# samuel-watson/glmmrMCML

Measured on AMD Instinct MI355X. Metric: MCML iters/sec x m chains (simlik evals/sec), higher is better.
Workload: dtype f64

## Files before the change

### glmmrmcml_amd/csrc/band_plan.h

```cpp
#pragma once
#include "common.h"
#include <algorithm>
#include <map>
#include <memory>

namespace mcml {

constexpr int BD_BM = 80, BD_BN = 128, BD_BK = 32, BD_STAGES = 3;
constexpr int BD_A_BYTES = BD_BK * BD_BM * 8;
constexpr int BD_B_BYTES = BD_BK * BD_BN * 8;
constexpr int BD_STAGE_BYTES = BD_A_BYTES + BD_B_BYTES;
constexpr size_t BD_LDS_BYTES = (size_t)BD_STAGES * BD_STAGE_BYTES;
constexpr int BD_NA = 3, BD_NB = 4, BD_PER_TILE = BD_NA + BD_NB;
constexpr int BD_TILE_ELEMS = BD_BM * BD_BN;

struct BandItem { int band, kt0, kt1, slot; };
struct BandRed { int band, s0, s1, pad; };

struct BandPlanDev {
    int gn = 0, nwg = 0, nred = 0, nslots = 0;
    int paired = 0;
    DevBuf items, wg_ptr, red, part;
};

struct SkinnyPlan {
    int nrb = 0, nkc = 0, ldp = 0;
    DevBuf range;
    DevBuf part;
};

struct BandPlan {
    int M = 0, K = 0, nbands = 0;
    std::vector<int> kr;
    long tiles = 0;
    std::map<int, std::unique_ptr<BandPlanDev>> by_gn;
    std::unique_ptr<SkinnyPlan> skinny;

    void reset(int M_, int K_, const std::vector<int>& kr_)
    {
        M = M_; K = K_; kr = kr_; nbands = (M + BD_BM - 1) / BD_BM;
        tiles = 0;
        for (int b = 0; b < nbands; ++b) tiles += kr[2 * b + 1] - kr[2 * b];
        by_gn.clear();
        skinny.reset();
    }

    static bool decompose(const std::vector<int>& kr, int nbands, int gn, int target_wg, std::vector<BandItem>& items,
                          std::vector<int>& wg_ptr, std::vector<BandRed>& red, int& nslots)
    {
        items.clear(); wg_ptr.clear(); red.clear(); nslots = 0;
        const int npairs = (nbands + 1) / 2;
        if ((long)npairs * gn * 5 >= (long)target_wg * 4) {
            for (int p = 0; p < npairs; ++p) {
                wg_ptr.push_back((int)items.size());
                items.push_back({p, kr[2 * p], kr[2 * p + 1], -1});
                const int q = nbands - 1 - p;
                if (q > p) items.push_back({q, kr[2 * q], kr[2 * q + 1], -1});
            }
            wg_ptr.push_back((int)items.size());
            return true;
        }
        int nwg = target_wg / gn; if (nwg < 1) nwg = 1;
        constexpr long OVH = 3;
        auto fill = [&](long cap, bool emit) -> int {
            int used = 1; long room = cap;
            if (emit) wg_ptr.push_back(0);
            for (int b = 0; b < nbands; ++b) {
                int k0 = kr[2 * b]; const int k1 = kr[2 * b + 1];
                const int first = (int)items.size();
                int pieces = 0;
                do {
                    if (room < OVH + 2) { ++used; room = cap; if (emit) wg_ptr.push_back((int)items.size()); }
                    long take = (room - OVH) / 2; if (take > k1 - k0) take = k1 - k0;
                    if (emit) items.push_back({b, k0, k0 + (int)take, -1});
                    k0 += (int)take; room -= OVH + 2 * take; ++pieces;
                } while (k0 < k1);
                if (emit && pieces > 1) {
                    for (int t = 0; t < pieces; ++t) items[first + t].slot = nslots + t;
                    red.push_back({b, nslots, nslots + pieces, 0});
                    nslots += pieces;
                }
            }
            if (emit) wg_ptr.push_back((int)items.size());
            return used;
        };
        long T = 0;
        for (int b = 0; b < nbands; ++b) T += kr[2 * b + 1] - kr[2 * b];
        long lo = OVH + 2, hi = 2 * T + OVH * nbands + OVH + 2;
        while (lo < hi) {
            const long mid = (lo + hi) / 2;
            if (fill(mid, false) <= nwg) hi = mid; else lo = mid + 1;
        }
        fill(lo, true);
        return false;
    }

    int device_plan(int gn, hipStream_t s, BandPlanDev** out)
    {
        auto it = by_gn.find(gn);
        if (it != by_gn.end()) { *out = it->second.get(); return MCML_OK; }
        std::unique_ptr<BandPlanDev> d(new BandPlanDev());
        std::vector<BandItem> items; std::vector<int> wg_ptr; std::vector<BandRed> red; int nslots = 0;
        d->paired = decompose(kr, nbands, gn, 256, items, wg_ptr, red, nslots) ? 1 : 0;
        d->gn = gn; d->nwg = (int)wg_ptr.size() - 1; d->nred = (int)red.size(); d->nslots = nslots;
        MCML_TRY(d->items.ensure(sizeof(BandItem) * (items.size() + 1)));
        MCML_TRY(d->wg_ptr.ensure(sizeof(int) * wg_ptr.size()));
        MCML_HIP(hipMemcpyAsync(d->items.p, items.data(), sizeof(BandItem) * items.size(), hipMemcpyHostToDevice, s));
        MCML_HIP(hipMemcpyAsync(d->wg_ptr.p, wg_ptr.data(), sizeof(int) * wg_ptr.size(), hipMemcpyHostToDevice, s));
        if (nslots > 0) {
            MCML_TRY(d->red.ensure(sizeof(BandRed) * red.size()));
            MCML_HIP(hipMemcpyAsync(d->red.p, red.data(), sizeof(BandRed) * red.size(), hipMemcpyHostToDevice, s));
            MCML_TRY(d->part.ensure(sizeof(double) * (size_t)nslots * gn * BD_TILE_ELEMS));
        }
        MCML_HIP(hipStreamSynchronize(s));
        *out = d.get();
        by_gn[gn] = std::move(d);
        return MCML_OK;
    }
};

}
```

### glmmrmcml_amd/csrc/debug_hooks.hip

```cpp
#include "dgemm_mfma.h"
#include "dgemm_dl.h"
#include "dgemm_band.h"

using namespace mcml;

extern "C" int glmmr_mcml_dbg_dgemm(int M, int N, int K, const double* A, int lda,
                                    const double* B, int ldb, int b_nmajor,
                                    double alpha, double beta, double* C, int ldc,
                                    int lower_only, int force_tile)
{
    int ndev = 0;
    if (hipGetDeviceCount(&ndev) != hipSuccess || ndev == 0) {
        set_error("no HIP device: libglmmr_mcml_hip has no CPU fallback");
        return MCML_ENODEVICE;
    }
    hipStream_t s = nullptr;
    DevMat dA, dB, dC;
    if (force_tile == 40) {
        MCML_REQUIRE(!b_nmajor && !lower_only, "dbg_dgemm: the direct-to-LDS kernel takes a K-major B and all tiles");
        const int kpad = round_up(K, 32);
        MCML_TRY(dA.alloc(M, K, 32));
        MCML_HIP(hipMemset(dA.d(), 0, sizeof(double) * (size_t)dA.ld * dA.cols_alloc));
        MCML_HIP(hipMemcpy2D(dA.d(), sizeof(double) * dA.ld, A, sizeof(double) * lda, sizeof(double) * M, K, hipMemcpyHostToDevice));
        MCML_TRY(dB.alloc(kpad, N));
// ... 45 lines not shown
    auto rnd = [&]() { x ^= x << 13; x ^= x >> 7; x ^= x << 17; return (double)(x >> 11) / 9007199254740992.0 * 2 - 1; };
    for (auto& v : hA) v = rnd();
    for (auto& v : hB) v = rnd();
    DevMat dA, dB, dC;
    MCML_TRY(upload_matrix(dA, hA.data(), M, K, M, s));
    if (b_nmajor) MCML_TRY(upload_matrix(dB, hB.data(), N, K, N, s));
    else MCML_TRY(upload_matrix(dB, hB.data(), K, N, K, s));
    MCML_TRY(upload_matrix(dC, hC.data(), M, N, M, s));
    EpiAxpby epi{dC.d(), dC.ld, beta != 0.0 ? 1e-3 : 1.0, beta};
    const bool lo = lower_only != 0;
    auto go = [&]() {
        if (force_tile >= 20)
            return b_nmajor ? launch_gemm_dl<true>(s, M, N, K, dA.d(), dA.ld, dB.d(), dB.ld, epi, lo, force_tile - 19)
                            : launch_gemm_dl<false>(s, M, N, K, dA.d(), dA.ld, dB.d(), dB.ld, epi, lo, force_tile - 19);
        return b_nmajor ? launch_gemm<true>(s, M, N, K, dA.d(), dA.ld, dB.d(), dB.ld, epi, lo, force_tile)
                        : launch_gemm<false>(s, M, N, K, dA.d(), dA.ld, dB.d(), dB.ld, epi, lo, force_tile);
    };
    for (int i = 0; i < 3; i++) MCML_TRY(go());
    hipEvent_t e0, e1;
    MCML_HIP(hipEventCreate(&e0));
    MCML_HIP(hipEventCreate(&e1));
    MCML_HIP(hipEventRecord(e0, s));
    for (int i = 0; i < iters; i++) MCML_TRY(go());
    MCML_HIP(hipEventRecord(e1, s));
    MCML_HIP(hipEventSynchronize(e1));
    float ms = 0;
    MCML_HIP(hipEventElapsedTime(&ms, e0, e1));
    *ms_per_launch = ms / iters;
    (void)hipEventDestroy(e0);
    (void)hipEventDestroy(e1);
    return MCML_OK;
}

extern "C" int glmmr_mcml_dbg_dgemm_band(int M, int N, int K, const double* A, int lda, const double* B, int ldb,
                                         double* C, int ldc, int* tiles_executed)
{
    int ndev = 0;
    if (hipGetDeviceCount(&ndev) != hipSuccess || ndev == 0) {
        set_error("no HIP device: libglmmr_mcml_hip has no CPU fallback");
        return MCML_ENODEVICE;
    }
    MCML_REQUIRE(M > 0 && N > 0 && K > 0 && A && B && C, "dbg_dgemm_band: bad argument");
    hipStream_t s = nullptr;
    DevMat dA, dB, dC;
    MCML_TRY(dA.alloc(M, K, 32));
    MCML_HIP(hipMemset(dA.d(), 0, sizeof(double) * (size_t)dA.ld * dA.cols_alloc));
    MCML_HIP(hipMemcpy2D(dA.d(), sizeof(double) * dA.ld, A, sizeof(double) * lda, sizeof(double) * M, K, hipMemcpyHostToDevice));
    MCML_TRY(dB.alloc(round_up(K, 32), N));
    MCML_HIP(hipMemset(dB.d(), 0, sizeof(double) * (size_t)dB.ld * N));
    MCML_HIP(hipMemcpy2D(dB.d(), sizeof(double) * dB.ld, B, sizeof(double) * ldb, sizeof(double) * K, N, hipMemcpyHostToDevice));
    MCML_TRY(dC.alloc(M, N));
    MCML_HIP(hipMemset(dC.d(), 0, sizeof(double) * (size_t)dC.ld * N));
    MCML_REQUIRE(dlds_applicable(M, N, K, dA.d(), dA.ld, dA.cols_alloc, dB.d(), dB.ld), "dbg_dgemm_band: contract");
    const int nbands = (M + BD_BM - 1) / BD_BM;
    DevBuf kr;
    MCML_TRY(kr.ensure(sizeof(int) * 2 * nbands));
    hipLaunchKernelGGL(k_band_ranges, dim3(nbands), dim3(256), 0, s, dA.d(), dA.ld, M, K, kr.as<int>());
    MCML_HIP(hipGetLastError());
    std::vector<int> hk(2 * nbands);
    MCML_HIP(hipMemcpy(hk.data(), kr.p, sizeof(int) * 2 * nbands, hipMemcpyDeviceToHost));
    BandPlan plan;
    plan.reset(M, K, hk);
    if (tiles_executed) *tiles_executed = (int)plan.tiles;
    EpiAxpby epi{dC.d(), dC.ld, 1.0, 0.0};
    MCML_TRY(launch_gemm_band(s, plan, N, dA.d(), dA.ld, dB.d(), dB.ld, epi));
    MCML_TRY(download_matrix(C, ldc, dC.d(), dC.ld, M, N, s));
    return MCML_OK;
}

extern "C" int glmmr_mcml_dbg_band_clocks(int M, int N, int iters, int mode, double* out3)
{
    int ndev = 0;
    if (hipGetDeviceCount(&ndev) != hipSuccess || ndev == 0) {
        set_error("no HIP device: libglmmr_mcml_hip has no CPU fallback");
        return MCML_ENODEVICE;
    }
    hipStream_t s = nullptr;
    if (getenv("GLMMR_MCML_DBG_STREAM")) MCML_HIP(hipStreamCreateWithFlags(&s, hipStreamNonBlocking));
    std::vector<double> hA((size_t)M * M, 0.0), hB((size_t)M * N);
    uint64_t x = 88172645463325252ULL;
    auto rnd = [&]() { x ^= x << 13; x ^= x >> 7; x ^= x << 17; return (double)(x >> 11) / 9007199254740992.0 * 2 - 1; };
    const bool cst = getenv("GLMMR_MCML_DBG_DATA") && !strcmp(getenv("GLMMR_MCML_DBG_DATA"), "const");
    const bool dec = getenv("GLMMR_MCML_DBG_DATA") && !strcmp(getenv("GLMMR_MCML_DBG_DATA"), "decay");
    for (int j = 0; j < M; ++j) for (int i = j; i < M; ++i) hA[i + (size_t)j * M] = cst ? 1.0 : dec ? rnd() * std::exp(-(double)(i - j) / 40.0) : rnd();
    for (auto& v : hB) v = cst ? 1.0 : rnd();
    DevMat dA, dB, dC;
    MCML_TRY(dA.alloc(M, M, 32));
    MCML_HIP(hipMemset(dA.d(), 0, sizeof(double) * (size_t)dA.ld * dA.cols_alloc));
    MCML_HIP(hipMemcpy2D(dA.d(), sizeof(double) * dA.ld, hA.data(), sizeof(double) * M, sizeof(double) * M, M, hipMemcpyHostToDevice));
    MCML_TRY(dB.alloc(round_up(M, 32), N));
    MCML_HIP(hipMemset(dB.d(), 0, sizeof(double) * (size_t)dB.ld * N));
    MCML_HIP(hipMemcpy2D(dB.d(), sizeof(double) * dB.ld, hB.data(), sizeof(double) * M, sizeof(double) * M, N, hipMemcpyHostToDevice));
    MCML_TRY(dC.alloc(M, N));
    const int nbands = (M + BD_BM - 1) / BD_BM;
    DevBuf kr, clk;
    MCML_TRY(kr.ensure(sizeof(int) * 2 * nbands));
    MCML_TRY(clk.ensure(16));
    MCML_HIP(hipMemset(clk.p, 0, 16));
    hipLaunchKernelGGL(k_band_ranges, dim3(nbands), dim3(256), 0, s, dA.d(), dA.ld, M, M, kr.as<int>());
    std::vector<int> hk(2 * nbands);
    MCML_HIP(hipMemcpy(hk.data(), kr.p, sizeof(int) * 2 * nbands, hipMemcpyDeviceToHost));
    BandPlan plan;
    plan.reset(M, M, hk);
    const double tiles = (double)plan.tiles;
    EpiAxpby epi{dC.d(), dC.ld, 1.0, 0.0};
    if (mode < 0) {
        for (int i = 0; i < 3; i++)
            MCML_TRY((launch_gemm_band<EpiAxpby, false>(s, plan, N, dA.d(), dA.ld, dB.d(), dB.ld, epi)));
        hipEvent_t f0, f1;
        MCML_HIP(hipEventCreate(&f0));
        MCML_HIP(hipEventCreate(&f1));
        MCML_HIP(hipEventRecord(f0, s));
        for (int i = 0; i < iters; i++)
            MCML_TRY((launch_gemm_band<EpiAxpby, false>(s, plan, N, dA.d(), dA.ld, dB.d(), dB.ld, epi)));
        MCML_HIP(hipEventRecord(f1, s));
        MCML_HIP(hipEventSynchronize(f1));
        float fms = 0;
        MCML_HIP(hipEventElapsedTime(&fms, f0, f1));
        out3[0] = fms / iters; out3[1] = 0;
        out3[2] = 2.0 * 80.0 * 32.0 * tiles * N / (fms / iters * 1e-3) / 1e12;
        (void)hipEventDestroy(f0);
        (void)hipEventDestroy(f1);
        return MCML_OK;
    }
    if (mode & 16) {
        BandPlanDev* d = nullptr;
        MCML_TRY(plan.device_plan((N + BD_BN - 1) / BD_BN, s, &d));
        const int nb = d->nwg * d->gn;
        DevBuf st;
        MCML_TRY(st.ensure(sizeof(unsigned long long) * (8 + 8 * (size_t)nb)));
        for (int rep = 0; rep < 3; ++rep) {
            MCML_HIP(hipMemset(st.p, 0, sizeof(unsigned long long) * (8 + 8 * (size_t)nb)));
            MCML_TRY((launch_gemm_band<EpiAxpby, true>(s, plan, N, dA.d(), dA.ld, dB.d(), dB.ld, epi, st.as<unsigned long long>(), mode)));
            MCML_HIP(hipDeviceSynchronize());
        }
        std::vector<unsigned long long> h(8 + 8 * (size_t)nb);
// ... 167 lines not shown
```

### glmmrmcml_amd/csrc/dgemm_band.h

```cpp
#pragma once
#include "dgemm_dlds.h"
#include "band_plan.h"

namespace mcml {

struct BandP {
    GemmP g;
    const BandItem* items;
    const int* wg_ptr;
    int nwg;
    double* part;
    int mode;
    unsigned long long* clocks;
};

static __global__ __launch_bounds__(256) void k_band_ranges(const double* A, int lda, int M, int K, int* krange)
{
    __shared__ int smin[256], smax[256];
    const int band = blockIdx.x, r0 = band * BD_BM;
    const int rows = (M - r0 < BD_BM) ? (M - r0) : BD_BM;
    int kmin = 1 << 30, kmax = -1;
    for (int k = threadIdx.x; k < K; k += 256) {
        const double* col = A + r0 + (size_t)k * lda;
        bool nz = false;
        for (int r = 0; r < rows; ++r) nz |= (col[r] != 0.0);
        if (nz) { kmin = min(kmin, k); kmax = max(kmax, k); }
    }
    smin[threadIdx.x] = kmin; smax[threadIdx.x] = kmax;
    __syncthreads();
    for (int o = 128; o > 0; o >>= 1) {
        if ((int)threadIdx.x < o) {
            smin[threadIdx.x] = min(smin[threadIdx.x], smin[threadIdx.x + o]);
            smax[threadIdx.x] = max(smax[threadIdx.x], smax[threadIdx.x + o]);
        }
        __syncthreads();
    }
    if (threadIdx.x == 0) {
        if (smax[0] < 0) { krange[2 * band] = 0; krange[2 * band + 1] = 0; }
        else { krange[2 * band] = smin[0] / BD_BK; krange[2 * band + 1] = smax[0] / BD_BK + 1; }
    }
}

#if defined(__HIP_DEVICE_COMPILE__)
#define BD_RD(dst, addr, off) asm volatile("ds_read_b64 %0, %1 offset:%2" : "=v"(dst) : "v"(addr), "i"(off))
#else
#define BD_RD(dst, addr, off) (dst = 0.0)
#endif
template <int KS>
__device__ __forceinline__ void bd_read(double (&a)[5], double& b, unsigned aaddr, unsigned baddr)
{
    BD_RD(a[0], aaddr, KS * 4 * BD_BM * 8);
    BD_RD(a[1], aaddr, KS * 4 * BD_BM * 8 + 128);
    BD_RD(a[2], aaddr, KS * 4 * BD_BM * 8 + 256);
    BD_RD(a[3], aaddr, KS * 4 * BD_BM * 8 + 384);
    BD_RD(a[4], aaddr, KS * 4 * BD_BM * 8 + 512);
    BD_RD(b, baddr, KS * 2 * BD_BN * 16);
}
template <int LEAVE>
__device__ __forceinline__ void bd_wait(double (&a)[5], double& b)
{
#if defined(__HIP_DEVICE_COMPILE__)
    if constexpr (LEAVE == 6)
        asm volatile("s_waitcnt lgkmcnt(6)" : "+v"(a[0]), "+v"(a[1]), "+v"(a[2]), "+v"(a[3]), "+v"(a[4]), "+v"(b));
    else
        asm volatile("s_waitcnt lgkmcnt(0)" : "+v"(a[0]), "+v"(a[1]), "+v"(a[2]), "+v"(a[3]), "+v"(a[4]), "+v"(b));
#endif
}
__device__ __forceinline__ void bd_mfma(d4 (&acc)[5][1], const double (&a)[5], double b)
{
#pragma unroll
    for (int i = 0; i < 5; ++i) acc[i][0] = __builtin_amdgcn_mfma_f64_16x16x4f64(b, a[i], acc[i][0], 0, 0, 0);
}
// ... 1 lines not shown
template <class Epi, bool DBG>
__global__ __launch_bounds__(512) void dgemm_band_kernel(BandP bp, Epi epi)
{
    const GemmP& p = bp.g;
    extern __shared__ __attribute__((aligned(16))) double smem[];
    char* lds = reinterpret_cast<char*>(smem);
    const int tid = threadIdx.x, lane = tid & 63, wave = __builtin_amdgcn_readfirstlane(tid >> 6);
    const int l15 = lane & 15, lk = lane >> 4;
    unsigned long long t0c = 0, t0r = 0;
    if constexpr (DBG)
        if (bp.clocks && blockIdx.x == 0 && tid == 0) { t0c = __builtin_amdgcn_s_memtime(); t0r = __builtin_amdgcn_s_memrealtime(); }

    const int nblk = bp.nwg * p.gn;
    const int bid = blockIdx.x;
    const int q8 = nblk >> 3, r8 = nblk & 7, xcd = bid & 7;
    const int nid = (xcd < r8 ? xcd * (q8 + 1) : r8 * (q8 + 1) + (xcd - r8) * q8) + (bid >> 3);
    const int pw = nid / p.gn, bj = nid - pw * p.gn;
    const int n0 = bj * BD_BN;

    unsigned vob[BD_NB]; int lb[BD_NB];
#pragma unroll
    for (int s = 0; s < BD_NB; ++s) {
        const int c = wave + 8 * s;
        const int kp = c >> 1, n = ((c & 1) << 6) + lane;
        int gn = n0 + n;
        if (gn >= p.N) gn = 0;
        vob[s] = (unsigned)((2 * kp + (size_t)gn * p.ldb) * 8);
        lb[s] = BD_A_BYTES + c * 1024;
    }
    const size_t stepA = (size_t)BD_BK * p.lda * 8;

    const int it0 = bp.wg_ptr[pw], it1 = bp.wg_ptr[pw + 1];
    BandItem item{0, 0, 0, -1};
    int m0 = 0;
    unsigned voa[BD_NA]; int la[BD_NA];
#pragma unroll
    for (int s = 0; s < BD_NA; ++s) {
        int c = wave + 8 * s;
        if (c >= 20) c = wave + 8;
        la[s] = c * 1024;
    }
    const char* sA = nullptr; const char* sB = nullptr;
    auto load_item = [&](int it) {
#if defined(__HIP_DEVICE_COMPILE__)
        {
            typedef int i4s __attribute__((ext_vector_type(4)));
            i4s raw;
            const BandItem* ip = bp.items + it;
            asm volatile("s_load_dwordx4 %0, %1, 0x0\n\ts_waitcnt lgkmcnt(0)" : "=&s"(raw) : "s"(ip) : "memory");
            item.band = raw.x; item.kt0 = raw.y; item.kt1 = raw.z; item.slot = raw.w;
        }
#else
        item = bp.items[it];
#endif
        m0 = item.band * BD_BM;
#pragma unroll
        for (int s = 0; s < BD_NA; ++s) {
            int c = wave + 8 * s;
            if (c >= 20) c = wave + 8;
            const int o = c * 1024 + lane * 16;
            const int k = o / (BD_BM * 8), m = (o - k * BD_BM * 8) >> 3;
            int gm = m0 + m;
            if (gm >= p.M) gm = 0;
            voa[s] = (unsigned)((gm + (size_t)k * p.lda) * 8);
        }
        sA = reinterpret_cast<const char*>(p.A) + (size_t)item.kt0 * stepA;
        sB = reinterpret_cast<const char*>(p.B) + (size_t)item.kt0 * (BD_BK * 8);
    };
    auto issue = [&](int stage) {
#if defined(__HIP_DEVICE_COMPILE__)
        const unsigned lbase = (unsigned)(size_t)(lds_ptr_t)lds + stage * BD_STAGE_BYTES;
#pragma unroll
        for (int s = 0; s < BD_NA; ++s)
            asm volatile("s_mov_b32 m0, %0\n\ts_nop 0\n\tglobal_load_lds_dwordx4 %1, %2"
                         :: "s"(lbase + la[s]), "v"(voa[s]), "s"(sA) : "memory", "m0");
#pragma unroll
        for (int s = 0; s < BD_NB; ++s)
            asm volatile("s_mov_b32 m0, %0\n\ts_nop 0\n\tglobal_load_lds_dwordx4 %1, %2"
                         :: "s"(lbase + lb[s]), "v"(vob[s]), "s"(sB) : "memory", "m0");
        sA += stepA;
        sB += BD_BK * 8;
#else
        (void)stage; (void)stepA; (void)sA; (void)sB;
#endif
    };
    auto wait_leave = [&](int tiles) {
        static_assert(BD_PER_TILE == 7, "vmcnt immediates below");
        if (tiles >= 2) asm volatile("s_waitcnt vmcnt(14)" ::: "memory");
        else if (tiles == 1) asm volatile("s_waitcnt vmcnt(7)" ::: "memory");
        else asm volatile("s_waitcnt vmcnt(0)" ::: "memory");
    };
    const int mode = DBG ? (bp.mode & 15) : 0;
    const bool stamps = DBG && (bp.mode & 16) && bp.clocks;
    auto stamp = [&](int i) {
        if constexpr (DBG)
            if (stamps && tid == 0) bp.clocks[8 + 8 * (size_t)blockIdx.x + i] = __builtin_amdgcn_s_memrealtime();
    };
    stamp(0);
    bool first_item = true;
    bool pre = false;
    int issued = 0;
    if (it0 < it1) load_item(it0);
    for (int it = it0; it < it1;) {
        const int band = item.band, e_m0 = m0, slot = item.slot;
        const int nk = item.kt1 - item.kt0;

        d4 acc[5][1];
#pragma unroll
        for (int i = 0; i < 5; ++i) acc[i][0] = d4{0.0, 0.0, 0.0, 0.0};

        if (nk > 0 && mode == 0) {
            const unsigned lds0 = (unsigned)(size_t)(lds_ptr_t)lds;
            const unsigned aoff = lds0 + lk * (BD_BM * 8) + l15 * 8;
            const unsigned boff = lds0 + BD_A_BYTES + (((lk >> 1) * BD_BN + wave * 16 + l15) << 4) + ((lk & 1) << 3);
            if (!pre) { issued = 0; for (; issued < BD_STAGES - 1 && issued < nk; ++issued) issue(issued); }
            wait_leave(issued - 1);
            __builtin_amdgcn_s_barrier();
            if (first_item) stamp(1);
            int st = 0;
            double ra[2][5], rb[2];
            bd_read<0>(ra[0], rb[0], aoff, boff);
            for (int kt = 0; kt < nk; ++kt) {
                if (issued < nk) {
                    int sn = st + BD_STAGES - 1; if (sn >= BD_STAGES) sn -= BD_STAGES;
                    issue(sn);
                    ++issued;
                }
                const unsigned aaddr = aoff + st * BD_STAGE_BYTES, baddr = boff + st * BD_STAGE_BYTES;
                int stn = st + 1; if (stn >= BD_STAGES) stn = 0;
#define BD_STEP(KS, CUR, NXT)                                   \
                bd_read<KS + 1>(ra[NXT], rb[NXT], aaddr, baddr); \
                bd_wait<6>(ra[CUR], rb[CUR]);                    \
                bd_mfma(acc, ra[CUR], rb[CUR]);                  \
                __builtin_amdgcn_sched_barrier(0);
                BD_STEP(0, 0, 1) BD_STEP(1, 1, 0) BD_STEP(2, 0, 1) BD_STEP(3, 1, 0)
                BD_STEP(4, 0, 1) BD_STEP(5, 1, 0) BD_STEP(6, 0, 1)
#undef BD_STEP
                wait_leave(issued - kt - 2);
                bd_wait<0>(ra[1], rb[1]);
                __builtin_amdgcn_s_barrier();
                if (kt + 1 < nk) bd_read<0>(ra[0], rb[0], aoff + stn * BD_STAGE_BYTES, boff + stn * BD_STAGE_BYTES);
                bd_mfma(acc, ra[1], rb[1]);
                __builtin_amdgcn_sched_barrier(0);
                st = stn;
            }
        } else if (DBG && nk > 0 && mode == 8) {
            int issued = 0;
            for (; issued < BD_STAGES - 1 && issued < nk; ++issued) issue(issued);
            wait_leave(issued - 1);
            __builtin_amdgcn_s_barrier();
            int st = 0;
            for (int kt = 0; kt < nk; ++kt) {
                if (issued < nk) {
                    int sn = st + BD_STAGES - 1; if (sn >= BD_STAGES) sn -= BD_STAGES;
                    issue(sn);
                    ++issued;
                }
                const double* as = reinterpret_cast<const double*>(lds + st * BD_STAGE_BYTES);
                const double* bs = reinterpret_cast<const double*>(lds + st * BD_STAGE_BYTES + BD_A_BYTES);
#pragma unroll
                for (int ks = 0; ks < BD_BK / 4; ++ks) {
                    const int kk = 4 * ks + lk;
                    double a[5];
#pragma unroll
                    for (int i = 0; i < 5; ++i) a[i] = as[kk * BD_BM + 16 * i + l15];
                    const double b = bs[((kk >> 1) * BD_BN + wave * 16 + l15) * 2 + (kk & 1)];
#pragma unroll
                    for (int i = 0; i < 5; ++i)
                        acc[i][0] = __builtin_amdgcn_mfma_f64_16x16x4f64(b, a[i], acc[i][0], 0, 0, 0);
                }
                wait_leave(issued - kt - 2);
                __builtin_amdgcn_s_barrier();
                st = st + 1; if (st >= BD_STAGES) st = 0;
            }
        } else if (DBG && nk > 0) {
            int issued = 0;
            if (!(mode & 1)) {
                for (; issued < BD_STAGES - 1 && issued < nk; ++issued) issue(issued);
// ... 19 lines not shown
                        b = bs[((kk >> 1) * BD_BN + wave * 16 + l15) * 2 + (kk & 1)];
                    }
#pragma unroll
                    for (int i = 0; i < 5; ++i)
                        acc[i][0] = __builtin_amdgcn_mfma_f64_16x16x4f64(b, a[i], acc[i][0], 0, 0, 0);
                }
                if (!(mode & 1)) wait_leave(issued - kt - 2);
                if (!(mode & 2)) __builtin_amdgcn_s_barrier();
                st = st + 1; if (st >= BD_STAGES) st = 0;
            }
        }
        if (first_item) stamp(2);
        ++it;
        pre = false;
        if (it < it1) {
            load_item(it);
            const int nkn = item.kt1 - item.kt0;
            if (mode == 0 && nk > 0 && nkn > 0) {
                issued = 0;
                for (; issued < BD_STAGES - 1 && issued < nkn; ++issued) issue(issued);
                pre = true;
            }
        }
        if (slot < 0) {
            epi(acc, e_m0, n0 + wave * 16, lane, p.M, p.N, band);
        } else {
            double* P = bp.part + ((size_t)slot * p.gn + bj) * BD_TILE_ELEMS + (size_t)wave * (20 * 64) + lane;
#pragma unroll
            for (int i = 0; i < 5; ++i)
#pragma unroll
                for (int r = 0; r < 4; ++r) P[(i * 4 + r) * 64] = acc[i][0][r];
        }
        if (first_item) { stamp(3); first_item = false; }
        if (!pre) __builtin_amdgcn_s_barrier();
    }
    if constexpr (DBG)
        if (stamps) { asm volatile("s_waitcnt vmcnt(0)" ::: "memory"); stamp(4); }
    if constexpr (DBG)
        if (bp.clocks && blockIdx.x == 0 && tid == 0) {
            atomicAdd(bp.clocks, __builtin_amdgcn_s_memtime() - t0c);
            atomicAdd(bp.clocks + 1, __builtin_amdgcn_s_memrealtime() - t0r);
        }
}

template <class Epi>
__global__ __launch_bounds__(128) void k_band_reduce(const BandRed* red, const double* part, int gn, int M, int N, Epi epi)
{
    const BandRed rd = red[blockIdx.x];
    const int bj = blockIdx.y;
    const int lane = threadIdx.x & 63, wave = blockIdx.z * 2 + (threadIdx.x >> 6);
    d4 acc[5][1];
#pragma unroll
    for (int i = 0; i < 5; ++i) acc[i][0] = d4{0.0, 0.0, 0.0, 0.0};
    const size_t pstride = (size_t)gn * BD_TILE_ELEMS;
    const double* P0 = part + ((size_t)rd.s0 * gn + bj) * BD_TILE_ELEMS + (size_t)wave * (20 * 64) + lane;
    for (int s = rd.s0; s < rd.s1; s += 4) {
        double v[4][20];
#pragma unroll
        for (int u = 0; u < 4; ++u) {
            const double* P = P0 + (size_t)(s - rd.s0 + (s + u < rd.s1 ? u : 0)) * pstride;
#pragma unroll
            for (int t = 0; t < 20; ++t) v[u][t] = P[t * 64];
        }
#pragma unroll
        for (int u = 0; u < 4; ++u)
            if (s + u < rd.s1) {
#pragma unroll
                for (int i = 0; i < 5; ++i)
#pragma unroll
                    for (int r = 0; r < 4; ++r) acc[i][0][r] += v[u][i * 4 + r];
            }
    }
    epi(acc, rd.band * BD_BM, bj * BD_BN + wave * 16, lane, M, N, rd.band);
}

template <class Epi, bool DBG = false>
static inline int launch_gemm_band(hipStream_t s, BandPlan& plan, int N, const double* A, int lda,
                                   const double* B, int ldb, const Epi& epi,
                                   unsigned long long* clocks = nullptr, int mode = 0)
{
    const int gn = (N + BD_BN - 1) / BD_BN;
    BandPlanDev* d = nullptr;
    MCML_TRY(plan.device_plan(gn, s, &d));
    BandP bp;
    bp.clocks = clocks;
    bp.mode = mode;
    bp.g = GemmP{plan.M, N, plan.K, A, lda, B, ldb, 0, gn, 0};
    bp.items = d->items.as<BandItem>();
    bp.wg_ptr = d->wg_ptr.as<int>();
    bp.nwg = d->nwg;
    bp.part = d->part.d();
    MCML_TRY(ensure_dynamic_lds(reinterpret_cast<const void*>(&dgemm_band_kernel<Epi, DBG>), (int)BD_LDS_BYTES));
    hipLaunchKernelGGL((dgemm_band_kernel<Epi, DBG>), dim3(d->nwg * gn), dim3(512), BD_LDS_BYTES, s, bp, epi);
    if (d->nred > 0)
        hipLaunchKernelGGL((k_band_reduce<Epi>), dim3(d->nred, gn, 4), dim3(128), 0, s, d->red.as<BandRed>(),
                           d->part.d(), gn, plan.M, N, epi);
    MCML_HIP(hipGetLastError());
    return MCML_OK;
}


}
```

### glmmrmcml_amd/csrc/model.hip

```cpp
#include "ctx.h"
#include "dgemm_mfma.h"
#include "dgemm_band.h"
#include "glm.h"
#include "reduce.h"

namespace mcml {

int model_setup(Ctx& c, const double* Z, const double* X, const double* y)
{
    const int n = c.n, Q = c.Q, P = c.P;
    MCML_TRY(upload_matrix(c.Z, Z, n, Q, n, c.stream));
    MCML_TRY(upload_matrix(c.X, X, n, P, n, c.stream));
    MCML_TRY(c.y.ensure(sizeof(double) * (size_t)pad_ld(n)));
    MCML_TRY(c.xb.ensure(sizeof(double) * (size_t)pad_ld(n)));
    MCML_HIP(hipMemsetAsync(c.y.p, 0, sizeof(double) * (size_t)pad_ld(n), c.stream));
    MCML_HIP(hipMemsetAsync(c.xb.p, 0, sizeof(double) * (size_t)pad_ld(n), c.stream));
    std::vector<double> yy(y, y + n);
    if (c.flink == 8)
        for (auto& v : yy) v = log(v);
    MCML_TRY(copy_h2d(c.y.p, yy.data(), sizeof(double) * n, c.stream));
    size_t nnz = 0; int maxrow = 0;
    std::vector<int> cnt(n, 0);
    for (int j = 0; j < Q; ++j)
        for (int i = 0; i < n; ++i)
// ... 216 lines not shown
    if (!c.sp.built) MCML_TRY(sparse_zl_setup(c));
    if (c.sp.possible && !c.no_sparse_zl && !c.l_foreign && c.L.ld == pad_ld(c.Q)) {
        const long tot = (long)c.n * c.sp.W;
        hipLaunchKernelGGL(k_ell_fill, dim3((unsigned)((tot + 255) / 256)), dim3(256), 0, c.stream,
                           c.sp.ell_src.as<int>(), c.sp.ell_z.d(), c.L.d(), tot, c.sp.ell_val.d());
        MCML_TRY(c.sp.csr_val.ensure(sizeof(double) * (size_t)(c.sp.nnz + 1)));
        hipLaunchKernelGGL(k_csr_fill, dim3((unsigned)((c.sp.nnz + 255) / 256)), dim3(256), 0, c.stream,
                           c.sp.csr_pos.as<int>(), c.sp.ell_val.d(), c.sp.nnz, c.sp.csr_val.d());
        MCML_HIP(hipGetLastError());
        c.sp.active = true;
        return MCML_OK;
    }
    c.sp.active = false;
    if (c.ZL.rows != c.n || c.ZL.cols != c.Q || !c.ZL.d()) {
        MCML_TRY(c.ZL.alloc(c.n, c.Q, 32));
        MCML_TRY(c.ZLT.alloc(c.Q, c.n, 32));
        MCML_HIP(hipMemsetAsync(c.ZL.d(), 0, sizeof(double) * (size_t)c.ZL.ld * c.ZL.cols_alloc, c.stream));
        MCML_HIP(hipMemsetAsync(c.ZLT.d(), 0, sizeof(double) * (size_t)c.ZLT.ld * c.ZLT.cols_alloc, c.stream));
    }
    if (c.z_width > 0) {
        MCML_TRY(z_times(c, c.L.d(), c.L.ld, c.Q, c.ZL.d(), c.ZL.ld));
    } else {
        EpiAxpby epi{c.ZL.d(), c.ZL.ld, 1.0, 0.0};
        MCML_TRY(launch_gemm<false>(c.stream, c.n, c.Q, c.Q, c.Z.d(), c.Z.ld, c.L.d(), c.L.ld, epi));
    }
    hipLaunchKernelGGL(k_transpose, dim3((c.n + 31) / 32, (c.Q + 31) / 32), dim3(256), 0, c.stream, c.ZL.d(),
                       c.ZL.ld, c.n, c.Q, c.ZLT.d(), c.ZLT.ld);
    MCML_HIP(hipGetLastError());
    c.band_fwd = c.band_bwd = false;
    const char* env = getenv("GLMMR_MCML_GEMM");
    if (!(env && (!strcmp(env, "reg") || !strcmp(env, "dlds")))) {
        auto ranges = [&](const DevMat& A, int M, int K, BandPlan& plan, bool& use, long& ntiles) -> int {
            const int nb = (M + BD_BM - 1) / BD_BM;
            MCML_TRY(c.kr_scratch.ensure(sizeof(int) * 2 * (size_t)nb));
            hipLaunchKernelGGL(k_band_ranges, dim3(nb), dim3(256), 0, c.stream, A.d(), A.ld, M, K, c.kr_scratch.as<int>());
            MCML_HIP(hipGetLastError());
            std::vector<int> h(2 * (size_t)nb);
            MCML_TRY(copy_d2h(h.data(), c.kr_scratch.p, sizeof(int) * h.size(), c.stream));
            MCML_HIP(hipStreamSynchronize(c.stream));
            if (!(plan.M == M && plan.K == K && plan.kr == h))
                plan.reset(M, K, h);
            const long dense = (long)nb * ((K + BD_BK - 1) / BD_BK);
            use = (env && !strcmp(env, "band")) || plan.tiles * 5 <= dense * 4;
            ntiles = plan.tiles;
            return MCML_OK;
        };
        MCML_TRY(ranges(c.ZL, c.n, c.Q, c.plan_fwd, c.band_fwd, c.band_fwd_tiles));
        MCML_TRY(ranges(c.ZLT, c.Q, c.n, c.plan_bwd, c.band_bwd, c.band_bwd_tiles));
    }
    return MCML_OK;
}

template <int FL>
__global__ __launch_bounds__(256) void k_loglik(const double* ZU, int ldz, int n, int ncols, const double* xb,
                                                const double* y, double var_par, int flink_rt, double* partials)
{
    const int flink = FL ? FL : flink_rt;
    __shared__ double sh[4];
    int i = blockIdx.x * 256 + threadIdx.x;
    double acc = 0;
    if (i < n) {
        const double yi = y[i], xbi = xb[i];
        for (int j = blockIdx.y; j < ncols; j += gridDim.y)
            acc += glm_logpdf(yi, xbi + ZU[i + (size_t)j * ldz], var_par, flink);
    }
    double r = block_sum(acc, sh);
    if (threadIdx.x == 0) partials[blockIdx.y * gridDim.x + blockIdx.x] = r;
}

int model_loglik_sum(Ctx& c, double var_par, double* sum_out)
{
    MCML_TRY(model_update_zu(c));
    int gx = (c.n + 255) / 256, gy = c.niter < 64 ? c.niter : 64;
    MCML_TRY(c.partials.ensure(sizeof(double) * (size_t)(gx * gy + 16)));
// ... 133 lines not shown
```

### include/glmmr_mcml_c.h

```cpp
#ifndef GLMMR_MCML_C_H
#define GLMMR_MCML_C_H
#include <stdint.h>

#ifdef __cplusplus
extern "C" {
#endif

#define GLMMR_MCML_OK            0
#define GLMMR_MCML_EINVAL       -1
#define GLMMR_MCML_EUNSUPPORTED -2
#define GLMMR_MCML_ENOTPD       -3
#define GLMMR_MCML_ESINGULAR    -4
#define GLMMR_MCML_EHIP         -5
#define GLMMR_MCML_ENODEVICE    -6
#define GLMMR_MCML_ENOMEM       -7

const char* glmmr_mcml_last_error(void);


typedef struct glmmr_mcml_problem {
    const int32_t* cov;
    int            cov_rows;
    const double*  data;
    int            data_len;
// ... 180 lines not shown
int glmmr_mcml_dbg_theta_log(glmmr_mcml_ctx* ctx, int enable, double* out, int cap_rows, int* nrows);
int glmmr_mcml_dbg_emulate_world(glmmr_mcml_ctx* ctx, int world, int mode);
int glmmr_mcml_dbg_leaf_profile(glmmr_mcml_ctx* ctx, unsigned long long* out10);
int glmmr_mcml_dbg_la_probe(glmmr_mcml_ctx* ctx, const double* start, int nstart, int kind, const double* v,
                            double var_par, const double* par, int npar, double* out, double* v_out,
                            double* beta_out, double* sigma_out);
int glmmr_mcml_dbg_dgemm(int M, int N, int K, const double* A, int lda, const double* B, int ldb,
                         int b_nmajor, double alpha, double beta, double* C, int ldc,
                         int lower_only, int force_tile );
int glmmr_mcml_dbg_log_prob_grad(glmmr_mcml_ctx* ctx, const double* beta, double var_par, const double* V,
                                 int ncols, double* lp, double* G);
int glmmr_mcml_dbg_normals(uint64_t seed, uint32_t chain, uint32_t prop, uint32_t tag, int n, double* out);
int glmmr_mcml_dbg_minstd(uint32_t seed, int n, double* out);
typedef double (*glmmr_mcml_objective)(const double* x, int n, void* user);
int glmmr_mcml_dbg_bobyqa(glmmr_mcml_objective f, void* user, int n, const double* x0, const double* lower,
                          const double* upper, double rhobeg, double rhoend, int maxfun, double* x_out,
                          double* f_out, int* nfev_out);
int glmmr_mcml_dbg_bobyqa_batch(glmmr_mcml_objective f, void* user, int n, const double* x0, const double* lower,
                                const double* upper, double rhobeg, double rhoend, int maxfun, int width,
                                double* x_out, double* f_out, int* nfev_out, int* rounds_out);
typedef int (*glmmr_mcml_batch_objective)(const double* X, int n, int k, double* F, void* user);
int glmmr_mcml_dbg_bobyqa_rounds(glmmr_mcml_batch_objective fb, void* user, int n, const double* x0, const double* lower,
                                 const double* upper, double rhobeg, double rhoend, int maxfun, int width,
                                 double* x_out, double* f_out, int* nfev_out, int* rounds_out);
int glmmr_mcml_dbg_copy_roundtrip(const double* in, long long ld_in, double* out, long long ld_out, long long rows, long long cols);
int glmmr_mcml_dbg_fd_hessian(glmmr_mcml_objective f, void* user, int n, const double* x, double ndeps,
                              int usebounds, const double* lower, const double* upper, double* H);
int glmmr_mcml_dbg_dgemm_bench(int M, int N, int K, int b_nmajor, int iters, int force_tile,
                               double* ms_per_launch);
int glmmr_mcml_dbg_dgemm_bench2(int M, int N, int K, int b_nmajor, int iters, int force_tile, int lower_only,
                                double beta, double* ms_per_launch);
int glmmr_mcml_dbg_dgemm_band(int M, int N, int K, const double* A, int lda, const double* B, int ldb, double* C,
                              int ldc, int* tiles_executed);
int glmmr_mcml_dbg_band_clocks(int M, int N, int iters, int mode, double* out3);

#ifdef __cplusplus
}
#endif
#endif
```

Baseline: 1122.

## Skip zero MFMAs in band GEMM edge k-tiles using per-16-row sub-ranges

The band-range kernel now records, for each 16-row block of every 80-row band, the nonzero k range at 4-column granularity. The host turns these into per-item edge descriptors, loaded with a scalar dwordx16 load. Inside the k-loop, the leading and trailing k-tiles run a predicated path that issues each 16x16x4 MFMA only when its row block has nonzeros at that k-step. Interior tiles keep the unpredicated path. This cuts wasted MFMA work on the ragged edges of banded factors, at the cost of an extra edge load per item, branchy edge tiles, and a wider range kernel and readback.

```diff
diff --git a/glmmrmcml_amd/csrc/band_plan.h b/glmmrmcml_amd/csrc/band_plan.h
--- a/glmmrmcml_amd/csrc/band_plan.h
+++ b/glmmrmcml_amd/csrc/band_plan.h
@@ -13,14 +13,17 @@
 constexpr size_t BD_LDS_BYTES = (size_t)BD_STAGES * BD_STAGE_BYTES;
 constexpr int BD_NA = 3, BD_NB = 4, BD_PER_TILE = BD_NA + BD_NB;
 constexpr int BD_TILE_ELEMS = BD_BM * BD_BN;
+constexpr int BD_RB = BD_BM / 16, BD_KS = BD_BK / 4;
 
 struct BandItem { int band, kt0, kt1, slot; };
 struct BandRed { int band, s0, s1, pad; };
+struct BandEdge { int a, b, lo[BD_RB], hi[BD_RB], pad[4]; };
+static_assert(sizeof(BandEdge) == 64, "one s_load_dwordx16");
 
 struct BandPlanDev {
     int gn = 0, nwg = 0, nred = 0, nslots = 0;
     int paired = 0;
-    DevBuf items, wg_ptr, red, part;
+    DevBuf items, edges, wg_ptr, red, part;
 };
 
 struct SkinnyPlan {
@@ -32,17 +35,56 @@
 struct BandPlan {
     int M = 0, K = 0, nbands = 0;
     std::vector<int> kr;
+    std::vector<int> sub;
     long tiles = 0;
+    long mfmas = 0;
     std::map<int, std::unique_ptr<BandPlanDev>> by_gn;
     std::unique_ptr<SkinnyPlan> skinny;
 
-    void reset(int M_, int K_, const std::vector<int>& kr_)
+    void reset(int M_, int K_, const std::vector<int>& kr_, const std::vector<int>& sub_)
     {
-        M = M_; K = K_; kr = kr_; nbands = (M + BD_BM - 1) / BD_BM;
-        tiles = 0;
-        for (int b = 0; b < nbands; ++b) tiles += kr[2 * b + 1] - kr[2 * b];
+        M = M_; K = K_; kr = kr_; sub = sub_; nbands = (M + BD_BM - 1) / BD_BM;
+        tiles = mfmas = 0;
+        for (int b = 0; b < nbands; ++b) {
+            tiles += kr[2 * b + 1] - kr[2 * b];
+            mfmas += item_mfmas({b, kr[2 * b], kr[2 * b + 1], -1});
+        }
         by_gn.clear();
         skinny.reset();
+    }
+
+    BandEdge edge(const BandItem& x) const
+    {
+        BandEdge e{};
+        const int nk = x.kt1 - x.kt0, g0 = x.kt0 * BD_KS;
+        if (sub.empty()) {
+            e.a = 0; e.b = nk;
+            for (int i = 0; i < BD_RB; ++i) { e.lo[i] = 0; e.hi[i] = nk * BD_KS; }
+            return e;
+        }
+        int ke0 = 0, ke1 = 1 << 28;
+        for (int i = 0; i < BD_RB; ++i) {
+            const int lo = sub[2 * BD_RB * x.band + i], hi = sub[2 * BD_RB * x.band + BD_RB + i];
+            if (lo >= hi) { ke0 = ke1 = 0; }
+            else { ke0 = std::max(ke0, (lo + BD_KS - 1) / BD_KS); ke1 = std::min(ke1, hi / BD_KS); }
+            e.lo[i] = std::min(std::max(lo - g0, 0), nk * BD_KS);
+            e.hi[i] = std::min(std::max(hi - g0, e.lo[i]), nk * BD_KS);
+            if (lo >= hi) e.lo[i] = e.hi[i] = 0;
+        }
+        e.a = std::min(std::max(ke0 - x.kt0, 0), nk);
+        e.b = std::min(std::max(ke1 - x.kt0, e.a), nk);
+        return e;
+    }
+
+    long item_mfmas(const BandItem& x) const
+    {
+        const BandEdge e = edge(x);
+        long n = (long)(e.b - e.a) * BD_KS * BD_RB;
+        for (int i = 0; i < BD_RB; ++i) {
+            const int s0 = e.a * BD_KS, s1 = e.b * BD_KS;
+            n += std::max(0, std::min(e.hi[i], s0) - e.lo[i]) + std::max(0, e.hi[i] - std::max(e.lo[i], s1));
+        }
+        return n;
     }
 
     static bool decompose(const std::vector<int>& kr, int nbands, int gn, int target_wg, std::vector<BandItem>& items,
@@ -103,9 +145,13 @@
         std::vector<BandItem> items; std::vector<int> wg_ptr; std::vector<BandRed> red; int nslots = 0;
         d->paired = decompose(kr, nbands, gn, 256, items, wg_ptr, red, nslots) ? 1 : 0;
         d->gn = gn; d->nwg = (int)wg_ptr.size() - 1; d->nred = (int)red.size(); d->nslots = nslots;
+        std::vector<BandEdge> edges;
+        for (const BandItem& x : items) edges.push_back(edge(x));
         MCML_TRY(d->items.ensure(sizeof(BandItem) * (items.size() + 1)));
+        MCML_TRY(d->edges.ensure(sizeof(BandEdge) * (edges.size() + 1)));
         MCML_TRY(d->wg_ptr.ensure(sizeof(int) * wg_ptr.size()));
         MCML_HIP(hipMemcpyAsync(d->items.p, items.data(), sizeof(BandItem) * items.size(), hipMemcpyHostToDevice, s));
+        MCML_HIP(hipMemcpyAsync(d->edges.p, edges.data(), sizeof(BandEdge) * edges.size(), hipMemcpyHostToDevice, s));
         MCML_HIP(hipMemcpyAsync(d->wg_ptr.p, wg_ptr.data(), sizeof(int) * wg_ptr.size(), hipMemcpyHostToDevice, s));
         if (nslots > 0) {
             MCML_TRY(d->red.ensure(sizeof(BandRed) * red.size()));
diff --git a/glmmrmcml_amd/csrc/debug_hooks.hip b/glmmrmcml_amd/csrc/debug_hooks.hip
--- a/glmmrmcml_amd/csrc/debug_hooks.hip
+++ b/glmmrmcml_amd/csrc/debug_hooks.hip
@@ -101,8 +101,8 @@
     return MCML_OK;
 }
 
-extern "C" int glmmr_mcml_dbg_dgemm_band(int M, int N, int K, const double* A, int lda, const double* B, int ldb,
-                                         double* C, int ldc, int* tiles_executed)
+static int dbg_dgemm_band(int M, int N, int K, const double* A, int lda, const double* B, int ldb, double* C, int ldc,
+                          int subtile, int* tiles_executed, long long* mfmas, int* ranges)
 {
     int ndev = 0;
     if (hipGetDeviceCount(&ndev) != hipSuccess || ndev == 0) {
@@ -122,19 +122,40 @@
     MCML_HIP(hipMemset(dC.d(), 0, sizeof(double) * (size_t)dC.ld * N));
     MCML_REQUIRE(dlds_applicable(M, N, K, dA.d(), dA.ld, dA.cols_alloc, dB.d(), dB.ld), "dbg_dgemm_band: contract");
     const int nbands = (M + BD_BM - 1) / BD_BM;
-    DevBuf kr;
+    DevBuf kr, sub;
     MCML_TRY(kr.ensure(sizeof(int) * 2 * nbands));
-    hipLaunchKernelGGL(k_band_ranges, dim3(nbands), dim3(256), 0, s, dA.d(), dA.ld, M, K, kr.as<int>());
+    MCML_TRY(sub.ensure(sizeof(int) * 2 * BD_RB * nbands));
+    hipLaunchKernelGGL(k_band_ranges, dim3(nbands), dim3(256), 0, s, dA.d(), dA.ld, M, K, kr.as<int>(), sub.as<int>());
     MCML_HIP(hipGetLastError());
-    std::vector<int> hk(2 * nbands);
-    MCML_HIP(hipMemcpy(hk.data(), kr.p, sizeof(int) * 2 * nbands, hipMemcpyDeviceToHost));
+    std::vector<int> hk(2 * nbands), hs(2 * BD_RB * nbands);
+    MCML_HIP(hipMemcpy(hk.data(), kr.p, sizeof(int) * hk.size(), hipMemcpyDeviceToHost));
+    MCML_HIP(hipMemcpy(hs.data(), sub.p, sizeof(int) * hs.size(), hipMemcpyDeviceToHost));
+    if (ranges) {
+        for (int b = 0; b < nbands; ++b) {
+            ranges[(2 + 2 * BD_RB) * b] = hk[2 * b]; ranges[(2 + 2 * BD_RB) * b + 1] = hk[2 * b + 1];
+            for (int i = 0; i < 2 * BD_RB; ++i) ranges[(2 + 2 * BD_RB) * b + 2 + i] = hs[2 * BD_RB * b + i];
+        }
+    }
     BandPlan plan;
-    plan.reset(M, K, hk);
+    plan.reset(M, K, hk, subtile ? hs : std::vector<int>());
     if (tiles_executed) *tiles_executed = (int)plan.tiles;
+    if (mfmas) *mfmas = plan.mfmas * 8 * ((N + BD_BN - 1) / BD_BN);
     EpiAxpby epi{dC.d(), dC.ld, 1.0, 0.0};
     MCML_TRY(launch_gemm_band(s, plan, N, dA.d(), dA.ld, dB.d(), dB.ld, epi));
     MCML_TRY(download_matrix(C, ldc, dC.d(), dC.ld, M, N, s));
     return MCML_OK;
+}
+
+extern "C" int glmmr_mcml_dbg_dgemm_band(int M, int N, int K, const double* A, int lda, const double* B, int ldb,
+                                         double* C, int ldc, int* tiles_executed)
+{
+    return dbg_dgemm_band(M, N, K, A, lda, B, ldb, C, ldc, 1, tiles_executed, nullptr, nullptr);
+}
+
+extern "C" int glmmr_mcml_dbg_dgemm_band_edges(int M, int N, int K, const double* A, int lda, const double* B, int ldb,
+                                               double* C, int ldc, int subtile, long long* mfmas, int* ranges)
+{
+    return dbg_dgemm_band(M, N, K, A, lda, B, ldb, C, ldc, subtile, nullptr, mfmas, ranges);
 }
 
 extern "C" int glmmr_mcml_dbg_band_clocks(int M, int N, int iters, int mode, double* out3)
@@ -162,15 +183,18 @@
     MCML_HIP(hipMemcpy2D(dB.d(), sizeof(double) * dB.ld, hB.data(), sizeof(double) * M, sizeof(double) * M, N, hipMemcpyHostToDevice));
     MCML_TRY(dC.alloc(M, N));
     const int nbands = (M + BD_BM - 1) / BD_BM;
-    DevBuf kr, clk;
+    DevBuf kr, sub, clk;
     MCML_TRY(kr.ensure(sizeof(int) * 2 * nbands));
+    MCML_TRY(sub.ensure(sizeof(int) * 2 * BD_RB * nbands));
     MCML_TRY(clk.ensure(16));
     MCML_HIP(hipMemset(clk.p, 0, 16));
-    hipLaunchKernelGGL(k_band_ranges, dim3(nbands), dim3(256), 0, s, dA.d(), dA.ld, M, M, kr.as<int>());
-    std::vector<int> hk(2 * nbands);
-    MCML_HIP(hipMemcpy(hk.data(), kr.p, sizeof(int) * 2 * nbands, hipMemcpyDeviceToHost));
+    hipLaunchKernelGGL(k_band_ranges, dim3(nbands), dim3(256), 0, s, dA.d(), dA.ld, M, M, kr.as<int>(), sub.as<int>());
+    std::vector<int> hk(2 * nbands), hs(2 * BD_RB * nbands);
+    MCML_HIP(hipMemcpy(hk.data(), kr.p, sizeof(int) * hk.size(), hipMemcpyDeviceToHost));
+    MCML_HIP(hipMemcpy(hs.data(), sub.p, sizeof(int) * hs.size(), hipMemcpyDeviceToHost));
     BandPlan plan;
-    plan.reset(M, M, hk);
+    const char* stl = getenv("GLMMR_MCML_DBG_SUBTILE");
+    plan.reset(M, M, hk, (stl && !strcmp(stl, "0")) ? std::vector<int>() : hs);
     const double tiles = (double)plan.tiles;
     EpiAxpby epi{dC.d(), dC.ld, 1.0, 0.0};
     if (mode < 0) {
diff --git a/glmmrmcml_amd/csrc/dgemm_band.h b/glmmrmcml_amd/csrc/dgemm_band.h
--- a/glmmrmcml_amd/csrc/dgemm_band.h
+++ b/glmmrmcml_amd/csrc/dgemm_band.h
@@ -1,12 +1,14 @@
 #pragma once
 #include "dgemm_dlds.h"
 #include "band_plan.h"
+#include <type_traits>
 
 namespace mcml {
 
 struct BandP {
     GemmP g;
     const BandItem* items;
+    const BandEdge* edges;
     const int* wg_ptr;
     int nwg;
     double* part;
@@ -14,30 +16,46 @@
     unsigned long long* clocks;
 };
 
-static __global__ __launch_bounds__(256) void k_band_ranges(const double* A, int lda, int M, int K, int* krange)
-{
-    __shared__ int smin[256], smax[256];
+static __global__ __launch_bounds__(256) void k_band_ranges(const double* A, int lda, int M, int K, int* krange, int* sub)
+{
+    __shared__ int smin[BD_RB][256], smax[BD_RB][256];
     const int band = blockIdx.x, r0 = band * BD_BM;
     const int rows = (M - r0 < BD_BM) ? (M - r0) : BD_BM;
-    int kmin = 1 << 30, kmax = -1;
+    int kmin[BD_RB], kmax[BD_RB];
+#pragma unroll
+    for (int i = 0; i < BD_RB; ++i) { kmin[i] = 1 << 30; kmax[i] = -1; }
     for (int k = threadIdx.x; k < K; k += 256) {
         const double* col = A + r0 + (size_t)k * lda;
-        bool nz = false;
-        for (int r = 0; r < rows; ++r) nz |= (col[r] != 0.0);
-        if (nz) { kmin = min(kmin, k); kmax = max(kmax, k); }
-    }
-    smin[threadIdx.x] = kmin; smax[threadIdx.x] = kmax;
+#pragma unroll
+        for (int i = 0; i < BD_RB; ++i) {
+            bool nz = false;
+            for (int r = 16 * i; r < 16 * i + 16 && r < rows; ++r) nz |= (col[r] != 0.0);
+            if (nz) { kmin[i] = min(kmin[i], k); kmax[i] = max(kmax[i], k); }
+        }
+    }
+#pragma unroll
+    for (int i = 0; i < BD_RB; ++i) { smin[i][threadIdx.x] = kmin[i]; smax[i][threadIdx.x] = kmax[i]; }
     __syncthreads();
     for (int o = 128; o > 0; o >>= 1) {
         if ((int)threadIdx.x < o) {
-            smin[threadIdx.x] = min(smin[threadIdx.x], smin[threadIdx.x + o]);
-            smax[threadIdx.x] = max(smax[threadIdx.x], smax[threadIdx.x + o]);
+#pragma unroll
+            for (int i = 0; i < BD_RB; ++i) {
+                smin[i][threadIdx.x] = min(smin[i][threadIdx.x], smin[i][threadIdx.x + o]);
+                smax[i][threadIdx.x] = max(smax[i][threadIdx.x], smax[i][threadIdx.x + o]);
+            }
         }
         __syncthreads();
     }
     if (threadIdx.x == 0) {
-        if (smax[0] < 0) { krange[2 * band] = 0; krange[2 * band + 1] = 0; }
-        else { krange[2 * band] = smin[0] / BD_BK; krange[2 * band + 1] = smax[0] / BD_BK + 1; }
+        int bmin = 1 << 30, bmax = -1;
+        for (int i = 0; i < BD_RB; ++i) {
+            const bool any = smax[i][0] >= 0;
+            sub[2 * BD_RB * band + i] = any ? smin[i][0] / 4 : 0;
+            sub[2 * BD_RB * band + BD_RB + i] = any ? smax[i][0] / 4 + 1 : 0;
+            if (any) { bmin = min(bmin, smin[i][0]); bmax = max(bmax, smax[i][0]); }
+        }
+        if (bmax < 0) { krange[2 * band] = 0; krange[2 * band + 1] = 0; }
+        else { krange[2 * band] = bmin / BD_BK; krange[2 * band + 1] = bmax / BD_BK + 1; }
     }
 }
 
@@ -105,6 +123,7 @@
 
     const int it0 = bp.wg_ptr[pw], it1 = bp.wg_ptr[pw + 1];
     BandItem item{0, 0, 0, -1};
+    BandEdge edge{};
     int m0 = 0;
     unsigned voa[BD_NA]; int la[BD_NA];
 #pragma unroll
@@ -118,13 +137,20 @@
 #if defined(__HIP_DEVICE_COMPILE__)
         {
             typedef int i4s __attribute__((ext_vector_type(4)));
-            i4s raw;
+            typedef int i16s __attribute__((ext_vector_type(16)));
+            i4s raw; i16s re;
             const BandItem* ip = bp.items + it;
-            asm volatile("s_load_dwordx4 %0, %1, 0x0\n\ts_waitcnt lgkmcnt(0)" : "=&s"(raw) : "s"(ip) : "memory");
+            const BandEdge* ep = bp.edges + it;
+            asm volatile("s_load_dwordx4 %0, %2, 0x0\n\ts_load_dwordx16 %1, %3, 0x0\n\ts_waitcnt lgkmcnt(0)"
+                         : "=&s"(raw), "=&s"(re) : "s"(ip), "s"(ep) : "memory");
             item.band = raw.x; item.kt0 = raw.y; item.kt1 = raw.z; item.slot = raw.w;
+            edge.a = re[0]; edge.b = re[1];
+#pragma unroll
+            for (int i = 0; i < BD_RB; ++i) { edge.lo[i] = re[2 + i]; edge.hi[i] = re[2 + BD_RB + i]; }
         }
 #else
         item = bp.items[it];
+        edge = bp.edges[it];
 #endif
         m0 = item.band * BD_BM;
 #pragma unroll
@@ -159,9 +185,9 @@
     };
     auto wait_leave = [&](int tiles) {
         static_assert(BD_PER_TILE == 7, "vmcnt immediates below");
-        if (tiles >= 2) asm volatile("s_waitcnt vmcnt(14)" ::: "memory");
-        else if (tiles == 1) asm volatile("s_waitcnt vmcnt(7)" ::: "memory");
-        else asm volatile("s_waitcnt vmcnt(0)" ::: "memory");
+        if (tiles >= 2) __builtin_amdgcn_s_waitcnt(0xF70 | 14);
+        else if (tiles == 1) __builtin_amdgcn_s_waitcnt(0xF70 | 7);
+        else __builtin_amdgcn_s_waitcnt(0xF70);
     };
     const int mode = DBG ? (bp.mode & 15) : 0;
     const bool stamps = DBG && (bp.mode & 16) && bp.clocks;
@@ -193,7 +219,8 @@
             int st = 0;
             double ra[2][5], rb[2];
             bd_read<0>(ra[0], rb[0], aoff, boff);
-            for (int kt = 0; kt < nk; ++kt) {
+            auto ktile = [&](auto edge_t, int kt) {
+                constexpr bool EDGE = decltype(edge_t)::value;
                 if (issued < nk) {
                     int sn = st + BD_STAGES - 1; if (sn >= BD_STAGES) sn -= BD_STAGES;
                     issue(sn);
@@ -201,10 +228,21 @@
                 }
                 const unsigned aaddr = aoff + st * BD_STAGE_BYTES, baddr = boff + st * BD_STAGE_BYTES;
                 int stn = st + 1; if (stn >= BD_STAGES) stn = 0;
+                auto mfma = [&](int ks, const double (&a)[5], double b) {
+                    if constexpr (EDGE) {
+                        const int g = kt * BD_KS + ks;
+#pragma unroll
+                        for (int i = 0; i < 5; ++i)
+                            if (g >= edge.lo[i] && g < edge.hi[i])
+                                acc[i][0] = __builtin_amdgcn_mfma_f64_16x16x4f64(b, a[i], acc[i][0], 0, 0, 0);
+                    } else {
+                        bd_mfma(acc, a, b);
+                    }
+                };
 #define BD_STEP(KS, CUR, NXT)                                   \
                 bd_read<KS + 1>(ra[NXT], rb[NXT], aaddr, baddr); \
                 bd_wait<6>(ra[CUR], rb[CUR]);                    \
-                bd_mfma(acc, ra[CUR], rb[CUR]);                  \
+                mfma(KS, ra[CUR], rb[CUR]);                      \
                 __builtin_amdgcn_sched_barrier(0);
                 BD_STEP(0, 0, 1) BD_STEP(1, 1, 0) BD_STEP(2, 0, 1) BD_STEP(3, 1, 0)
                 BD_STEP(4, 0, 1) BD_STEP(5, 1, 0) BD_STEP(6, 0, 1)
@@ -213,10 +251,14 @@
                 bd_wait<0>(ra[1], rb[1]);
                 __builtin_amdgcn_s_barrier();
                 if (kt + 1 < nk) bd_read<0>(ra[0], rb[0], aoff + stn * BD_STAGE_BYTES, boff + stn * BD_STAGE_BYTES);
-                bd_mfma(acc, ra[1], rb[1]);
+                mfma(7, ra[1], rb[1]);
                 __builtin_amdgcn_sched_barrier(0);
                 st = stn;
-            }
+            };
+            int kt = 0;
+            for (; kt < edge.a; ++kt) ktile(std::true_type{}, kt);
+            for (; kt < edge.b; ++kt) ktile(std::false_type{}, kt);
+            for (; kt < nk; ++kt) ktile(std::true_type{}, kt);
         } else if (DBG && nk > 0 && mode == 8) {
             int issued = 0;
             for (; issued < BD_STAGES - 1 && issued < nk; ++issued) issue(issued);
@@ -302,6 +344,7 @@
                 for (int r = 0; r < 4; ++r) P[(i * 4 + r) * 64] = acc[i][0][r];
         }
         if (first_item) { stamp(3); first_item = false; }
+        __builtin_amdgcn_s_waitcnt(0xF70);
         if (!pre) __builtin_amdgcn_s_barrier();
     }
     if constexpr (DBG)
@@ -357,6 +400,7 @@
     bp.mode = mode;
     bp.g = GemmP{plan.M, N, plan.K, A, lda, B, ldb, 0, gn, 0};
     bp.items = d->items.as<BandItem>();
+    bp.edges = d->edges.as<BandEdge>();
     bp.wg_ptr = d->wg_ptr.as<int>();
     bp.nwg = d->nwg;
     bp.part = d->part.d();
diff --git a/glmmrmcml_amd/csrc/model.hip b/glmmrmcml_amd/csrc/model.hip
--- a/glmmrmcml_amd/csrc/model.hip
+++ b/glmmrmcml_amd/csrc/model.hip
@@ -272,14 +272,16 @@
     if (!(env && (!strcmp(env, "reg") || !strcmp(env, "dlds")))) {
         auto ranges = [&](const DevMat& A, int M, int K, BandPlan& plan, bool& use, long& ntiles) -> int {
             const int nb = (M + BD_BM - 1) / BD_BM;
-            MCML_TRY(c.kr_scratch.ensure(sizeof(int) * 2 * (size_t)nb));
-            hipLaunchKernelGGL(k_band_ranges, dim3(nb), dim3(256), 0, c.stream, A.d(), A.ld, M, K, c.kr_scratch.as<int>());
+            MCML_TRY(c.kr_scratch.ensure(sizeof(int) * (2 + 2 * BD_RB) * (size_t)nb));
+            hipLaunchKernelGGL(k_band_ranges, dim3(nb), dim3(256), 0, c.stream, A.d(), A.ld, M, K, c.kr_scratch.as<int>(),
+                               c.kr_scratch.as<int>() + 2 * nb);
             MCML_HIP(hipGetLastError());
-            std::vector<int> h(2 * (size_t)nb);
-            MCML_TRY(copy_d2h(h.data(), c.kr_scratch.p, sizeof(int) * h.size(), c.stream));
+            std::vector<int> hb((2 + 2 * BD_RB) * (size_t)nb);
+            MCML_TRY(copy_d2h(hb.data(), c.kr_scratch.p, sizeof(int) * hb.size(), c.stream));
             MCML_HIP(hipStreamSynchronize(c.stream));
-            if (!(plan.M == M && plan.K == K && plan.kr == h))
-                plan.reset(M, K, h);
+            const std::vector<int> h(hb.begin(), hb.begin() + 2 * nb), hs(hb.begin() + 2 * nb, hb.end());
+            if (!(plan.M == M && plan.K == K && plan.kr == h && plan.sub == hs))
+                plan.reset(M, K, h, hs);
             const long dense = (long)nb * ((K + BD_BK - 1) / BD_BK);
             use = (env && !strcmp(env, "band")) || plan.tiles * 5 <= dense * 4;
             ntiles = plan.tiles;
diff --git a/include/glmmr_mcml_c.h b/include/glmmr_mcml_c.h
--- a/include/glmmr_mcml_c.h
+++ b/include/glmmr_mcml_c.h
@@ -236,6 +236,8 @@
                                 double beta, double* ms_per_launch);
 int glmmr_mcml_dbg_dgemm_band(int M, int N, int K, const double* A, int lda, const double* B, int ldb, double* C,
                               int ldc, int* tiles_executed);
+int glmmr_mcml_dbg_dgemm_band_edges(int M, int N, int K, const double* A, int lda, const double* B, int ldb, double* C,
+                                    int ldc, int subtile, long long* mfmas, int* ranges);
 int glmmr_mcml_dbg_band_clocks(int M, int N, int iters, int mode, double* out3);
 
 #ifdef __cplusplus
```

Result: no change. 1130, median of 6 (+0.8%).
